# rskew/aiko_services

Measured on AMD Instinct MI355X. Metric: frames/sec (whole node) + p50 latency, ResNet-50 pipeline at 1/2/4/8 MI355X, higher is better.
Workload: dtype bf16; 1 GPU; global_batch=640, per_gpu_batch=640, parallelism=dp1, hipgraph=True, ingest=hbm, setup_frames=12, model=resnet50, pipeline=(SyntheticFrames ResNet50Classifier ClassifierTopK), gpu_lanes=2

## Files before the change

aiko_services_amd/csrc/bindings/conv.cpp:

```cpp
#include "checks.h"

namespace {

void conv_igemm_out(const at::Tensor& x, const c10::optional<at::Tensor>& x2, const at::Tensor& w,
                    const c10::optional<at::Tensor>& bias, const c10::optional<at::Tensor>& res,
                    at::Tensor& y, at::IntArrayRef geom, const c10::optional<at::Tensor>& zero) {
  TORCH_CHECK(geom.size() == 21 || geom.size() == 22, "aiko.conv_igemm_out: geom needs 21 or 22 ints");
  const int64_t variant = geom.size() == 22 ? geom[21] : 0;
  const int64_t H = geom[0], W = geom[1], C = geom[2], Cc = geom[3], R = geom[4], S = geom[5];
  const int64_t stride = geom[6], pad = geom[7], Ho = geom[8], Wo = geom[9], M = geom[10];
  const int64_t act = geom[11], ldy = geom[12], ldr = geom[13], bm = geom[14], bn = geom[15];
  const int64_t K1 = geom[16], H2 = geom[17], W2 = geom[18], C2 = geom[19], stride2 = geom[20];
  check_cuda_all({&x, &w, &y}, {"x", "w", "y"});
  TORCH_CHECK(x.scalar_type() == at::kBFloat16 && w.scalar_type() == at::kBFloat16 &&
                  y.scalar_type() == at::kBFloat16,
              "aiko.conv_igemm_out: x, w, y must be bfloat16");
  TORCH_CHECK(w.dim() == 2 && w.is_contiguous(), "aiko.conv_igemm_out: w must be [Cout, K] contiguous");
  const int64_t Cout = w.size(0), K = w.size(1);
  const bool dual = defined(x2);
  const int64_t Kmain = dual ? K1 : K;
  TORCH_CHECK(Kmain >= R * S * Cc && Kmain % 64 == 0 && Kmain - R * S * Cc < 64, "aiko.conv_igemm_out: K=",
              Kmain, " must be R*S*Cc rounded up to a multiple of 64");
  const void* x2ptr = nullptr;
  if (dual) {
    check_cuda(*x2, "x2");
    TORCH_CHECK(x2->scalar_type() == at::kBFloat16, "aiko.conv_igemm_out: x2 must be bf16");
    TORCH_CHECK((K - K1) % 64 == 0 && K - K1 <= C2 && C2 % 8 == 0 && K1 > 0,
                "aiko.conv_igemm_out: second source needs K-K1 (multiple of 64) <= C2");
    TORCH_CHECK(aligned(*x2, 16), "aiko.conv_igemm_out: x2 alignment");
    TORCH_CHECK(M % (Ho * Wo) == 0 && (Ho - 1) * stride2 < H2 && (Wo - 1) * stride2 < W2 &&
                    avail_elems(*x2) >= (M / (Ho * Wo)) * H2 * W2 * C2,
                "aiko.conv_igemm_out: x2 too small for the output geometry");
    x2ptr = x2->data_ptr();
  }
  TORCH_CHECK(Cc % 8 == 0 && (Cc <= C || C == 4), "aiko.conv_igemm_out: Cc must be a multiple of 8 within the pixel pitch (or span pixels of a 4-channel stem input)");
// ... 435 lines not shown
    dbg_ptr = reinterpret_cast<unsigned*>(dbg->data_ptr());
  }
  TORCH_CHECK(B * H * W * 256 < INT_MAX, "aiko.bneck_fused_out: batch too large for 32-bit pixel indices");
  check_launch(aiko_bneck_fused(x.data_ptr(), w1.data_ptr(), b1.data_ptr<float>(), w2.data_ptr(), b2.data_ptr<float>(),
                                w3.data_ptr(), b3.data_ptr<float>(), y.data_ptr(), (int)B, (int)H, (int)W, (int)cin,
                                (int)grid, dbg_ptr, cur_stream()),
               "bneck_fused");
}

void conv3x3_exp_out(const at::Tensor& t1, const at::Tensor& w2, const at::Tensor& b2, const at::Tensor& w3,
                     const at::Tensor& b3, const at::Tensor& res, at::Tensor& y, int64_t grid) {
  for (const at::Tensor* t : {&t1, &w2, &b2, &w3, &b3, &res, (const at::Tensor*)&y}) {
    check_cuda(*t, "conv3x3_exp operand");
    TORCH_CHECK(t->is_contiguous() && aligned(*t, 16),
                "aiko.conv3x3_exp_out: operands must be contiguous and 16-byte aligned");
  }
  for (const at::Tensor* t : {&t1, &w2, &w3, &res, (const at::Tensor*)&y})
    TORCH_CHECK(t->scalar_type() == at::kBFloat16, "aiko.conv3x3_exp_out: bf16 activations / weights");
  for (const at::Tensor* t : {&b2, &b3})
    TORCH_CHECK(t->scalar_type() == at::kFloat, "aiko.conv3x3_exp_out: fp32 biases");
  TORCH_CHECK(t1.dim() == 4 && t1.size(3) == 256, "aiko.conv3x3_exp_out: t1 must be [B, H, W, 256] NHWC");
  const int64_t B = t1.size(0), H = t1.size(1), W = t1.size(2);
  TORCH_CHECK(y.dim() == 4 && y.size(0) == B && y.size(1) == H && y.size(2) == W, "aiko.conv3x3_exp_out: y must be [B, H, W, N]");
  const int64_t N = y.size(3);
  TORCH_CHECK(N > 0 && N % 256 == 0, "aiko.conv3x3_exp_out: N must be a multiple of 256");
  TORCH_CHECK(res.sizes() == y.sizes(), "aiko.conv3x3_exp_out: res must have y's shape (identity residual)");
  TORCH_CHECK(w2.numel() == 256 * 9 * 256 && w2.size(0) == 256, "aiko.conv3x3_exp_out: w2 [256, 2304] (3x3, tap-major)");
  TORCH_CHECK(w3.numel() == N * 256, "aiko.conv3x3_exp_out: w3 must be the [N / 16, 8, 64, 8] fragment image");
  TORCH_CHECK(b2.numel() == 256 && b3.numel() == N, "aiko.conv3x3_exp_out: biases [256], [N]");
  TORCH_CHECK(y.data_ptr() != res.data_ptr() && y.data_ptr() != t1.data_ptr(), "aiko.conv3x3_exp_out: in place is not supported");
  TORCH_CHECK(grid >= 0, "aiko.conv3x3_exp_out: grid must be >= 0 (0: one workgroup per tile)");
  TORCH_CHECK(B > 0 && H > 0 && W > 0 && B * H * W * N * 2 < 0x7ffffff0LL,
              "aiko.conv3x3_exp_out: tensors too large for 32-bit offsets");
  check_launch(aiko_conv3x3_exp(t1.data_ptr(), w2.data_ptr(), b2.data_ptr<float>(), w3.data_ptr(), b3.data_ptr<float>(),
                                res.data_ptr(), y.data_ptr(), (int)B, (int)H, (int)W, (int)N, (int)grid, cur_stream()),
               "conv3x3_exp");
}

void stem_direct_out(const at::Tensor& frames, const at::Tensor& w, const c10::optional<at::Tensor>& bias,
                     at::Tensor& out, at::IntArrayRef geom, double fill, at::ArrayRef<double> mean,
                     at::ArrayRef<double> std, bool bgr) {
  check_cuda_all({&frames, &w, &out}, {"frames", "w", "out"});
  TORCH_CHECK(frames.scalar_type() == at::kByte && frames.dim() == 4 && frames.size(3) == 3 && frames.is_contiguous(),
              "aiko.stem_direct_out: frames must be uint8 [B, H, W, 3] contiguous");
  TORCH_CHECK(geom.size() == 10, "aiko.stem_direct_out: geom = [Ho, Wo, Hc, Wc, off_t, off_l, k, stride, pad, act]");
  const int64_t Ho = geom[0], Wo = geom[1], Hc = geom[2], Wc = geom[3], off_t = geom[4], off_l = geom[5];
  const int64_t k = geom[6], stride = geom[7], pad = geom[8], act = geom[9];
  TORCH_CHECK(off_t >= 0 && off_l >= 0 && off_t + Ho <= Hc && off_l + Wo <= Wc,
              "aiko.stem_direct_out: image must lie inside the canvas");
  const int64_t B = frames.size(0), Cout = out.size(3);
  const int64_t H1 = (Hc + 2 * pad - k) / stride + 1, W1 = (Wc + 2 * pad - k) / stride + 1;
  TORCH_CHECK(out.size(0) == B && out.size(1) == H1 && out.size(2) == W1, "aiko.stem_direct_out: out must be [B, ",
              H1, ", ", W1, ", Cout]");
  const int64_t ldo = pixel_pitch(out, "stem_direct_out");
  TORCH_CHECK(w.scalar_type() == at::kBFloat16 && w.is_contiguous() && w.dim() == 2 && w.size(0) == Cout &&
                  w.size(1) == 64 && k * k * 4 <= 64 && Cout % 16 == 0,
              "aiko.stem_direct_out: w bf16 [Cout, 64] contiguous (k <= 4, Cout % 16 == 0)");
  const float* bp = nullptr;
  if (defined(bias)) {
    check_cuda(*bias, "bias");
    TORCH_CHECK(bias->scalar_type() == at::kFloat && bias->numel() == Cout && bias->is_contiguous(), "aiko.stem_direct_out: bias fp32 [Cout]");
    bp = bias->data_ptr<float>();
  }
  TORCH_CHECK(mean.size() == 3 && std.size() == 3, "aiko.stem_direct_out: mean/std need 3 values");
  float m[3] = {(float)mean[0], (float)mean[1], (float)mean[2]};
  float s[3] = {(float)std[0], (float)std[1], (float)std[2]};
  check_launch(aiko_stem_direct(frames.data_ptr(), out.data_ptr(), w.data_ptr(), bp, B, frames.size(1),
                                frames.size(2), Ho, Wo, Hc, Wc, off_t, off_l, (float)fill, m, s, bgr ? 1 : 0, H1, W1,
// ... 73 lines not shown
```

aiko_services_amd/csrc/kernels/aiko_api.h:

```cpp
#pragma once

#include <hip/hip_runtime.h>

#include "conv_launch.h"

extern "C" {

int aiko_conv_igemm(const ConvLaunch* l);
int aiko_conv_glds(const ConvLaunch* l, const void* zero);
int aiko_conv_glds_tail(const void* x, const void* w, const float* bias, int H, int W, int C, int Cc, int R, int S,
                        int stride, int pad, int Ho, int Wo, int M, int K, int N, int act, const void* w2, const float* b2,
                        void* y2, int ldy2, int ldw2, int act2, const void* zero, const int* dec, void* boxes,
                        float* scores, int* cls, hipStream_t stream);
int aiko_conv_buf(const ConvLaunch* l, int occ, int mf32);
int aiko_conv_persist(const ConvLaunch* l);
int aiko_conv_wide(const ConvLaunch* l, int occ);

int aiko_conv_pw(const void* x, const void* w, const float* bias, const void* res, void* y, int M, int N,
                 int K, int ldx, int ldy, int ldr, int act, int cus, int mode, hipStream_t stream);
int aiko_conv_pw_dual(const void* x, const void* x2, const void* w, const float* bias, void* y, int M, int N,
                      int ldx, int ldx2, int ldy, int act, int Ho, int Wo, int H2, int W2, int s2, int cus,
                      hipStream_t stream);

int aiko_conv_narrow(const void* x, const void* w, const float* bias, const void* res, void* y, int H, int W, int C,
                     int Cc, int R, int S, int stride, int pad, int Ho, int Wo, int M, int Cout, int K, int act,
                     int ldy, int ldr, int th, int wreg, hipStream_t stream);

int aiko_conv3x3_patch(const void* x, const void* wimg, const float* bias, void* y, int B, int H, int W, int ldy,
                       int act, int grid, hipStream_t stream);
int aiko_conv3x3_patchw(const void* x, const void* wimg, const float* bias, void* y, int B, int H, int W, int ldx,
                        int ldy, int act, int grid, hipStream_t stream);
int aiko_conv3x3_rows(const void* x, const void* wimg, const float* bias, const void* res, void* y, int B, int H,
                      int W, int ldx, int ldy, int ldr, int act, int grid, hipStream_t stream);

int aiko_conv_chain(const void* A, const void* W1, const float* b1, const void* R, void* Y, const void* W2,
                    const float* b2, void* Z, const void* A2, int M, int K1, int N1, int N2, int grid,
                    hipStream_t stream);
int aiko_conv_chain2(const void* A, const void* W1, const float* b1, const void* R, void* Y, const void* W2,
                     const float* b2, void* Z, int M, int K1, int N1, int N2, int grid, hipStream_t stream);

int aiko_bneck_fused(const void* x, const void* w1, const float* b1, const void* w2, const float* b2,
                     const void* w3, const float* b3, void* y, int B, int H, int W, int cin, int grid,
                     unsigned* dbg, hipStream_t stream);
int aiko_conv3x3_exp(const void* t1, const void* w2, const float* b2, const void* w3img, const float* b3,
                     const void* res, void* y, int B, int H, int W, int N, int grid, hipStream_t stream);
int aiko_c2f_fused(const void* x, int ldx, const void* w1, const float* b1, int k1, const void* wa, const float* ba,
                   int ka, const void* wb, const float* bb, int kb, const void* w2, const float* b2, int k2, void* y, int ldy,
                   int B, int H, int W, int CI, int C, int CO, int shortcut, int rb, const void* xu, int ldxu, int cu, hipStream_t stream);
int aiko_c2f_bneck(const void* x, int ldx, const void* wa, const float* ba, int ka, const void* wb, const float* bb,
                   int kb, void* y, int ldy, int B, int H, int W, int C, int shortcut, int rb, hipStream_t stream);

int aiko_stem_pool(const void* x, const void* w, const float* bias, void* y, int B, int Hp, int Wp,
                   int Ho, int Wo, int Hm, int Wm, int ldy, int variant, hipStream_t stream);
int aiko_stem_pool_u8(const void* frames, const void* w, const float* bias, void* y, int B, int Hi, int Wi,
                      int Ho, int Wo, int Hm, int Wm, int ldy, const float* mean255, int variant, hipStream_t stream);

int aiko_resize_u8(const void* in, void* out, int B, int Hin, int Win, int Ho, int Wo, hipStream_t stream);
int aiko_batchnorm(const void* x, void* y, const float* scale, const float* shift, long P, int C, int ldx,
                   int ldy, int act, hipStream_t stream);
int aiko_preprocess(const void* in, void* out, int B, int Hin, int Win, int Ho, int Wo, int Hp,
                    int Wp, int pad_t, int pad_l, int Hc, int Wc, int off_t, int off_l, float fill,
                    const float* mean, const float* std, int bgr, hipStream_t stream);
int aiko_stem_direct(const void* in, void* out, const void* w, const float* bias, int B, int Hin, int Win,
                     int Ho, int Wo, int Hc, int Wc, int off_t, int off_l, float fill, const float* mean,
                     const float* std, int bgr, int H1, int W1, int Cout, int ldo, int k, int stride, int pad,
                     int act, hipStream_t stream);
int aiko_maxpool(const void* x, void* y, int B, int H, int W, int C, int Ho, int Wo, int k,
                 int s, int p, int ldx, int ldy, hipStream_t stream);
int aiko_mean_rows_f32(const void* x, float* y, int B, int T, int C, long ldb, hipStream_t stream);
int aiko_avgpool(const void* x, void* y, int B, int HW, int C, hipStream_t stream);
int aiko_softmax_topk(const void* logits, float* prob, int* index, int B, int N, int k,
                      hipStream_t stream);
int aiko_sppf_pool(void* x, int B, int H, int W, int ld, int c, int k, hipStream_t stream);
int aiko_zero_border_rows(void* x, int B, int rows, int C, hipStream_t stream);

int aiko_upsample2x(const void* x, void* y, int B, int H, int W, int C, int ldx, int ldy,
                    hipStream_t stream);
int aiko_yolo_decode(const void* const* feats, const int* H, const int* W, const int* strides,
// ... 114 lines not shown
```

aiko_services_amd/csrc/kernels/conv_exp.hip:

```cpp
#include <type_traits>

#include "conv_common.h"
#include "conv_wide_stage.h"
#include "aiko_api.h"

namespace aiko {

typedef __attribute__((ext_vector_type(2))) short i16x2;

__device__ __forceinline__ uint32_t relu_bf16x2(uint32_t v) {
  return __builtin_bit_cast(uint32_t, __builtin_elementwise_max(__builtin_bit_cast(i16x2, v), i16x2{0, 0}));
}

struct ConvExpParams {
  ConvParams c;
  const bf16_t* w3;
  const float* b3;
  int N;
};

__global__ __launch_bounds__(512, 1) void conv3x3_exp_kernel(ConvExpParams q) {
  const ConvParams& p = q.c;
  constexpr int BM = 256, BN = 256, BK = 64, WGN = 4, NW = 8, NS = 2;
  constexpr int WM = 128, WN = 64, MI = 8, NI = 4, NP = 2;
  constexpr int RPW = 8, RPI = 64, APT = 4, BPT = 4;
  constexpr int STAGE_ELEMS = (BM + BN) * BK;
  constexpr int T2_BLOCK = BM * 64;
  static_assert(NS * STAGE_ELEMS == 4 * T2_BLOCK, "the t2 slice fills the ring exactly");
  __shared__ __attribute__((aligned(16))) bf16_t ring[NS * STAGE_ELEMS];

  const int wave = __builtin_amdgcn_readfirstlane(threadIdx.x >> 6);
  const int wr = wave / WGN, wc = wave % WGN;
  const int ntiles = (p.M + BM - 1) / BM;
  const int G = gridDim.x;
  const int lid = xcd_remap(blockIdx.x, G);

  const __amdgpu_buffer_rsrc_t rx = wide_rsrc(p.x);
  const __amdgpu_buffer_rsrc_t rw = wide_rsrc(p.w);
  const __amdgpu_buffer_rsrc_t rw3 = wide_rsrc(q.w3);
  const int io_bytes = p.M * q.N * 2;
  const __amdgpu_buffer_rsrc_t rr =
      __builtin_amdgcn_make_buffer_rsrc(const_cast<bf16_t*>(p.res), (short)0, io_bytes, 0x00020000);
  const __amdgpu_buffer_rsrc_t ry = __builtin_amdgcn_make_buffer_rsrc(p.y, (short)0, io_bytes, 0x00020000);

  const int nkb = p.K / BK;
  const int nch = q.N / 128;

  for (int tile = lid; tile < ntiles; tile += G) {
    const int m0 = tile * BM;
    uint32_t lz = 0u;
    asm volatile("" : "+v"(lz));
    const int lane1 = __builtin_amdgcn_mbcnt_hi(~0u, __builtin_amdgcn_mbcnt_lo(~0u, lz));
    const int lrow = wave * RPW + (lane1 >> 3);
    const int lp = (lane1 & 7) ^ (lane1 >> 3);
    const int HoWo = p.Ho * p.Wo;
    uint32_t b_off[BPT];
#pragma unroll
    for (int i = 0; i < BPT; ++i) b_off[i] = (uint32_t)(((lrow + RPI * i) * p.K + lp * 8) * 2);

    const int fr = lane1 & 15, fq = lane1 >> 4;
    const int coff = ((fq & 1) << 4) | ((fq >> 1) << 3);
    const int sw = fr & 7;
// ... 110 lines not shown
      }
      if (kb < nkb) step(kb, S0{});
    }

    uint32_t lz2 = 0u;
    asm volatile("" : "+v"(lz2));
    const int lane2 = __builtin_amdgcn_mbcnt_hi(~0u, __builtin_amdgcn_mbcnt_lo(~0u, lz2));
    const int fr2 = lane2 & 15, fq2 = lane2 >> 4;
    const int coff2 = ((fq2 & 1) << 4) | ((fq2 >> 1) << 3);
    const int sw2 = fr2 & 7;
    const int x_r0 = (wr * WM + fr2) * 64;
    __syncthreads();
#pragma unroll
    for (int i = 0; i < MI; ++i) {
#pragma unroll
      for (int h = 0; h < NP; ++h) {
        f32x4 lo = acc[2 * h][i], hi = acc[2 * h + 1][i];
#pragma unroll
        for (int e = 0; e < 4; ++e) {
          const auto s = __builtin_amdgcn_permlane16_swap(__float_as_uint(lo[e]), __float_as_uint(hi[e]), false, false);
          lo[e] = __uint_as_float(s[0]);
          hi[e] = __uint_as_float(s[1]);
        }
        u32x4 o;
        o[0] = pack2(fmaxf(lo[0] + e_bias[h][0], 0.f), fmaxf(lo[1] + e_bias[h][1], 0.f));
        o[1] = pack2(fmaxf(lo[2] + e_bias[h][2], 0.f), fmaxf(lo[3] + e_bias[h][3], 0.f));
        o[2] = pack2(fmaxf(hi[0] + e_bias[h][4], 0.f), fmaxf(hi[1] + e_bias[h][5], 0.f));
        o[3] = pack2(fmaxf(hi[2] + e_bias[h][6], 0.f), fmaxf(hi[3] + e_bias[h][7], 0.f));
        const int piece = (h * 4 + (coff2 >> 3)) ^ sw2;
        *reinterpret_cast<u32x4*>(ring + wc * T2_BLOCK + (x_r0 + i * 16 * 64) + (piece << 3)) = o;
      }
    }

    const uint32_t row0 = (uint32_t)(((m0 + wr * WM + fr2) * q.N + wc * 32 + coff2) * 2);
    const uint32_t row_step = (uint32_t)(16 * q.N * 2);
    const uint32_t w_off = (uint32_t)(wc * 2 * 8 * 1024 + lane2 * 16);
    bf16x8 wreg[4][2];
    u32x4 e_res[2][MI];
    f32x2 e_b3[4];
    auto load_w = [&](int c, int ks) __attribute__((always_inline)) {
      const uint32_t base = c < nch ? w_off : kWideOOB;
#pragma unroll
      for (int j = 0; j < 2; ++j)
        wreg[ks & 3][j] = __builtin_bit_cast(bf16x8, __builtin_amdgcn_raw_buffer_load_b128(
            rw3, base, (uint32_t)c * 65536u + (uint32_t)((j * 8 + ks) * 1024), 0));
    };
    auto load_res = [&](int c, auto par_tag) __attribute__((always_inline)) {
      constexpr int P = decltype(par_tag)::value;
      const uint32_t cb = (uint32_t)c * 256u;
      const uint32_t base = c < nch ? row0 : kWideOOB;
      uint32_t rs = row_step;
      asm volatile("" : "+s"(rs));
#pragma unroll
      for (int i = 0; i < MI; ++i)
        e_res[P][i] = __builtin_bit_cast(u32x4, __builtin_amdgcn_raw_buffer_load_b128(
            rr, base + rs * i, cb, 0));
    };
    auto load_b3 = [&](int c) __attribute__((always_inline)) {
      const int n = c * 128 + wc * 32 + coff2;
      const f32x4 b0 = *reinterpret_cast<const f32x4*>(q.b3 + n);
      const f32x4 b1 = *reinterpret_cast<const f32x4*>(q.b3 + n + 4);
      e_b3[0] = f32x2{b0[0], b0[1]}; e_b3[1] = f32x2{b0[2], b0[3]};
      e_b3[2] = f32x2{b1[0], b1[1]}; e_b3[3] = f32x2{b1[2], b1[3]};
    };
    using P0 = std::integral_constant<int, 0>;
    using P1 = std::integral_constant<int, 1>;
// ... 47 lines not shown
#pragma unroll
        for (int e = 0; e < 4; ++e) {
          const auto s = __builtin_amdgcn_permlane16_swap(__float_as_uint(lo[e]), __float_as_uint(hi[e]), false, false);
          lo[e] = __uint_as_float(s[0]);
          hi[e] = __uint_as_float(s[1]);
        }
        const f32x2 v[4] = {f32x2{lo[0], lo[1]} + e_b3[0], f32x2{lo[2], lo[3]} + e_b3[1],
                            f32x2{hi[0], hi[1]} + e_b3[2], f32x2{hi[2], hi[3]} + e_b3[3]};
        u32x4 o;
#pragma unroll
        for (int e = 0; e < 4; ++e) {
          const f32x2 r = {__uint_as_float(e_res[P][i][e] << 16), __uint_as_float(e_res[P][i][e] & 0xffff0000u)};
          const f32x2 t = v[e] + r;
          o[e] = relu_bf16x2(pack2(t[0], t[1]));
        }
        __builtin_amdgcn_raw_buffer_store_b128(o, ry, row0 + rs * i, cb, 0);
        asm volatile("s_nop 1");
        __builtin_amdgcn_sched_barrier(0);
      }
      load_res(c + 2, par_tag);
    };
    for (int c = 0; c < nch; c += 2) {
      chunk(c, P0{});
      chunk(c + 1, P1{});
    }
    __syncthreads();
  }
}

}

extern "C" int aiko_conv3x3_exp(const void* t1, const void* w2, const float* b2, const void* w3img,
                                const float* b3, const void* res, void* y, int B, int H, int W, int N,
                                int grid, hipStream_t stream) {
  using namespace aiko;
  const long M = (long)B * H * W;
  if (N <= 0 || N % 256 || M <= 0 || M * N * 2 >= 0x7ffffff0L || H * W <= 0 || grid < 0) return -1;
  ConvExpParams q;
  ConvParams& p = q.c;
  p.x = static_cast<const bf16_t*>(t1);
  p.w = static_cast<const bf16_t*>(w2);
  p.bias = b2;
  p.res = static_cast<const bf16_t*>(res);
  p.y = static_cast<bf16_t*>(y);
  p.H = H; p.W = W; p.C = 256; p.Cc = 256; p.R = 3; p.S = 3;
  p.stride = 1; p.pad = 1; p.Ho = H; p.Wo = W; p.M = (int)M; p.Cout = 256; p.K = 9 * 256;
  p.act = 1; p.ldy = N; p.ldr = N;
  p.x2 = nullptr;
  p.K1 = p.K; p.H2 = 0; p.W2 = 0; p.C2 = 0; p.stride2 = 1;
  conv_params_finalize(p);
  q.w3 = static_cast<const bf16_t*>(w3img);
  q.b3 = b3;
  q.N = N;
  const int ntiles = (int)((M + 255) / 256);
  const int g = grid > 0 && grid < ntiles ? grid : ntiles;
  conv3x3_exp_kernel<<<dim3(g), 512, 0, stream>>>(q);
  return (int)hipGetLastError();
}
```

aiko_services_amd/csrc/kernels/conv_wide.hip:

```cpp
#include <cstdlib>
#include <type_traits>

#include "conv_common.h"
#include "conv_wide_stage.h"
#include "aiko_api.h"

namespace aiko {

template <int BM, int BN, int WGM, int WGN, int NS, bool RES_PF, int OCC, int BK = 64, int NR = 0>
__global__ __launch_bounds__(64 * WGM * WGN, OCC) void conv_wide_kernel(ConvParams p) {
  constexpr int NW = WGM * WGN;
  static_assert(NW == 4 || NW == 8, "4 or 8 waves");
  static_assert(BK == 64 || BK == 32, "64- or 32-deep K blocks");
  constexpr int PPR = BK / 8;
  constexpr int D = NS - 1;
  constexpr int BNR = NR ? NR : BN;
  static_assert(BNR <= BN && BNR % (16 * WGN) == 0, "exact-N tile");
  constexpr int WM = BM / WGM, WN = BNR / WGN;
  constexpr int MI = WM / 16, NI = WN / 16;
  static_assert((NR != 0 || NI % 2 == 0) && MI >= 1, "wave tile: whole 16-pixel blocks, channel blocks in pairs");
  constexpr bool TAIL = NI % 2 != 0;
  constexpr int RPW = 64 / PPR;
  constexpr int RPI = RPW * NW;
  static_assert(BM % RPI == 0 && BN % RPI == 0, "tile rows in whole DMA pieces");
// ... 282 lines not shown
      const f32x4 a = acc[NI - 1][i];
      uint2 r = {0u, 0u};
      if (p.res) {
        if constexpr (RES_PF) r = e_rtail[i];
        else r = *reinterpret_cast<const uint2*>(p.res + (size_t)m * p.ldr + ntail);
      }
      float v[4] = {a[0] + e_btail[0], a[1] + e_btail[1], a[2] + e_btail[2], a[3] + e_btail[3]};
      const float rv[4] = {__uint_as_float(r.x << 16), __uint_as_float(r.x & 0xffff0000u),
                           __uint_as_float(r.y << 16), __uint_as_float(r.y & 0xffff0000u)};
      if (p.res && !post) {
#pragma unroll
        for (int e = 0; e < 4; ++e) v[e] += rv[e];
      }
      if (act == 1) {
#pragma unroll
        for (int e = 0; e < 4; ++e) v[e] = fmaxf(v[e], 0.f);
      } else if (act == 2) {
#pragma unroll
        for (int e = 0; e < 4; ++e) v[e] = silu(v[e]);
      } else if (act == 3) {
#pragma unroll
        for (int e = 0; e < 4; ++e) v[e] = gelu_erf(v[e]);
      }
      if (p.res && post) {
#pragma unroll
        for (int e = 0; e < 4; ++e) v[e] += rv[e];
      }
      *reinterpret_cast<uint2*>(p.y + (size_t)m * p.ldy + ntail) = uint2{pack2(v[0], v[1]), pack2(v[2], v[3])};
    }
  }
}


template <int BM, int BN, int WGM, int WGN, int NS, bool RES = false>
__global__ __launch_bounds__(64 * WGM * WGN, 1) void conv_wide_pers_kernel(ConvParams p) {
  constexpr int BK = 64, PPR = 8;
  constexpr int NW = WGM * WGN;
  static_assert(NW == 8, "8 waves");
  static_assert(NS == 2 || NS == 3, "2- or 3-slot ring");
  constexpr int D = NS - 1;
  constexpr int WM = BM / WGM, WN = BN / WGN;
  constexpr int MI = WM / 16, NI = WN / 16, NP = NI / 2;
  static_assert(NI % 2 == 0, "channel blocks in pairs");
  constexpr int RPW = 64 / PPR, RPI = RPW * NW;
  static_assert(BM % RPI == 0 && BN % RPI == 0, "tile rows in whole DMA pieces");
  constexpr int APT = BM / RPI, BPT = BN / RPI, PER = APT + BPT;
  constexpr int NST = MI * NP;
  constexpr int STAGE_ELEMS = (BM + BN) * BK;
  constexpr int BIAS_FLOATS = 2048;
  static_assert(NS * STAGE_ELEMS * 2 + BIAS_FLOATS * 4 <= 160 * 1024, "LDS budget");
  __shared__ __attribute__((aligned(16))) bf16_t ring[NS * STAGE_ELEMS + BIAS_FLOATS * 2];
  float* const sbias = reinterpret_cast<float*>(ring + NS * STAGE_ELEMS);

  const int tid = threadIdx.x, lane = tid & 63;
  const int wave = __builtin_amdgcn_readfirstlane(tid >> 6);
  const int wr = wave / WGN, wc = wave % WGN;
  const int ntn = (p.Cout + BN - 1) / BN;
  const int ntiles = ((p.M + BM - 1) / BM) * ntn;
  const int G = gridDim.x;
  const int lid = xcd_remap(blockIdx.x, G);
  if (lid >= ntiles) return;
  const int nkb = p.K / BK;
  const int nblocks = ((ntiles - lid + G - 1) / G) * nkb;

  for (int c = tid; c < BIAS_FLOATS; c += 64 * NW) sbias[c] = (p.bias && c < p.Cout) ? p.bias[c] : 0.f;
  __syncthreads();

// ... 216 lines not shown
    }
    if constexpr (RES) {
      if (ckb == nkb - 1 - D) load_res(ct);
    }
    issue_next(std::integral_constant<int, PREV>{});
    compute(slot_tag);
    epi_prev2 = epi_prev;
    epi_prev = false;
    if (++ckb == nkb) {
      epilogue(ct);
      ct += G;
      ckb = 0;
      epi_prev = true;
    }
  };
  int g = 0;
  if constexpr (NS == 2) {
    for (; g + 2 <= nblocks; g += 2) {
      step(g, S0{});
      step(g + 1, S1{});
    }
    if (g < nblocks) step(g, S0{});
  } else {
    for (; g + 3 <= nblocks; g += 3) {
      step(g, S0{});
      step(g + 1, S1{});
      step(g + 2, S2{});
    }
    if (g < nblocks) step(g, S0{});
    if (g + 1 < nblocks) step(g + 1, S1{});
  }
  asm volatile("s_waitcnt vmcnt(0)" ::: "memory");
}
}

extern "C" int aiko_conv_wide(const ConvLaunch* l, int occ) {
  using namespace aiko;
  const int M = l->M, Cout = l->Cout, K = l->K, bm = l->bm, bn = l->bn;
  const void* res = l->res;
  hipStream_t stream = l->stream;
  if (l->Cc % 64 || l->R * l->S > 32 || l->R > 16 || l->S > 16 || (l->x2 && (K - l->K1) % 64) || Cout % 8) return -1;
  const ConvParams p = conv_params(*l);
  dim3 grid(((M + bm - 1) / bm) * ((Cout + bn - 1) / bn));
  if (occ == 18) {
    if (Cout % 16) return -1;
    if (bm == 256 && bn == 80)
      conv_wide_kernel<256, 128, 8, 1, 2, true, 1, 64, 80><<<grid, 512, 0, stream>>>(p);
    else if (bm == 128 && bn == 80)
      conv_wide_kernel<128, 128, 8, 1, 2, true, 2, 64, 80><<<grid, 512, 0, stream>>>(p);
    else if (bm == 256 && bn == 144)
      conv_wide_kernel<256, 192, 8, 1, 2, true, 1, 64, 144><<<grid, 512, 0, stream>>>(p);
    else if (bm == 128 && bn == 144)
      conv_wide_kernel<128, 192, 8, 1, 2, true, 1, 64, 144><<<grid, 512, 0, stream>>>(p);
    else
      return -1;
  } else if (occ == 20) {
    if (Cout > 2048 || (res != nullptr && K < 192)) return -1;
    int dev = 0, cus = 0;
    (void)hipGetDevice(&dev);
    if (hipDeviceGetAttribute(&cus, hipDeviceAttributeMultiprocessorCount, dev) != hipSuccess || cus <= 0) cus = 256;
    const char* cap = getenv("AIKO_CONV_PERS_GRID");
    if (cap && atoi(cap) > 0) cus = atoi(cap);
    const int ntiles = (int)grid.x;
    dim3 pg(ntiles < cus ? ntiles : cus);
    const bool r = res != nullptr;
    if (bm == 256 && bn == 256 && !r)
      conv_wide_pers_kernel<256, 256, 2, 4, 2><<<pg, 512, 0, stream>>>(p);
    else if (bm == 256 && bn == 128 && !r)
      conv_wide_pers_kernel<256, 128, 4, 2, 3><<<pg, 512, 0, stream>>>(p);
    else if (bm == 128 && bn == 256 && !r)
      conv_wide_pers_kernel<128, 256, 2, 4, 3><<<pg, 512, 0, stream>>>(p);
    else if (bm == 256 && bn == 128)
      conv_wide_pers_kernel<256, 128, 4, 2, 3, true><<<pg, 512, 0, stream>>>(p);
    else if (bm == 128 && bn == 256)
      conv_wide_pers_kernel<128, 256, 2, 4, 3, true><<<pg, 512, 0, stream>>>(p);
    else
      return -1;
  } else if (occ == 19) {
    if (bm == 128 && bn == 128)
      conv_wide_kernel<128, 128, 2, 2, 2, true, 2><<<grid, 256, 0, stream>>>(p);
    else if (bm == 128 && bn == 256)
      conv_wide_kernel<128, 256, 2, 2, 3, true, 1><<<grid, 256, 0, stream>>>(p);
    else
      return -1;
  } else if (occ <= 1) {
    if (bm == 256 && bn == 256)
      conv_wide_kernel<256, 256, 2, 4, 2, false, 1><<<grid, 512, 0, stream>>>(p);
    else if (bm == 256 && bn == 128)
      conv_wide_kernel<256, 128, 4, 2, 3, true, 1><<<grid, 512, 0, stream>>>(p);
    else if (bm == 128 && bn == 256)
      conv_wide_kernel<128, 256, 2, 4, 3, true, 1><<<grid, 512, 0, stream>>>(p);
    else if (bm == 256 && bn == 64)
      conv_wide_kernel<256, 64, 4, 2, 3, true, 1><<<grid, 512, 0, stream>>>(p);
    else if (bm == 128 && bn == 128)
      conv_wide_kernel<128, 128, 2, 4, 3, true, 1><<<grid, 512, 0, stream>>>(p);
    else
      return -1;
  } else if (occ == 11) {
    if (bm == 256 && bn == 256)
      conv_wide_kernel<256, 256, 2, 4, 4, false, 1, 32><<<grid, 512, 0, stream>>>(p);
    else if (bm == 256 && bn == 128)
      conv_wide_kernel<256, 128, 4, 2, 4, true, 1, 32><<<grid, 512, 0, stream>>>(p);
    else if (bm == 128 && bn == 256)
      conv_wide_kernel<128, 256, 2, 4, 4, true, 1, 32><<<grid, 512, 0, stream>>>(p);
    else
      return -1;
  } else {
    if (bm == 128 && bn == 128)
// ... 15 lines not shown
```

Baseline: 101,200 frames/s.

## Add register-resident t2 schedule for fused 3x3+expand conv second GEMM

Adds a templated P2REG variant of the fused conv3x3+1x1-expand kernel that loads each wave's t2 activation slice into registers once. The expand weights are then streamed into the LDS ring in double-buffered halves via DMA, and the bias is staged in shared memory. This reorganizes the second GEMM so every wave covers 32 pixel rows across all output channels, aiming to cut repeated LDS activation reads and overlap weight loads with MFMA work. It is enabled by default through an env-var switch for N<=4096, at the cost of more register pressure and extra LDS for the bias.

```diff
diff --git a/aiko_services_amd/csrc/bindings/conv.cpp b/aiko_services_amd/csrc/bindings/conv.cpp
--- a/aiko_services_amd/csrc/bindings/conv.cpp
+++ b/aiko_services_amd/csrc/bindings/conv.cpp
@@ -1,6 +1,8 @@
 #include "checks.h"
 
 namespace {
+
+constexpr int kExpP2Default = 1;
 
 void conv_igemm_out(const at::Tensor& x, const c10::optional<at::Tensor>& x2, const at::Tensor& w,
                     const c10::optional<at::Tensor>& bias, const c10::optional<at::Tensor>& res,
@@ -502,8 +504,14 @@
   TORCH_CHECK(grid >= 0, "aiko.conv3x3_exp_out: grid must be >= 0 (0: one workgroup per tile)");
   TORCH_CHECK(B > 0 && H > 0 && W > 0 && B * H * W * N * 2 < 0x7ffffff0LL,
               "aiko.conv3x3_exp_out: tensors too large for 32-bit offsets");
+  const char* p2 = getenv("AIKO_EXP_P2");
+  int sched = p2 && *p2 ? atoi(p2) : kExpP2Default;
+  TORCH_CHECK(sched == 0 || sched == 1, "aiko.conv3x3_exp_out: AIKO_EXP_P2 must be 0 or 1");
+  if (!(p2 && *p2) && N > 4096) sched = 0;
+  TORCH_CHECK(sched == 0 || N <= 4096, "aiko.conv3x3_exp_out: AIKO_EXP_P2=1 needs N <= 4096");
   check_launch(aiko_conv3x3_exp(t1.data_ptr(), w2.data_ptr(), b2.data_ptr<float>(), w3.data_ptr(), b3.data_ptr<float>(),
-                                res.data_ptr(), y.data_ptr(), (int)B, (int)H, (int)W, (int)N, (int)grid, cur_stream()),
+                                res.data_ptr(), y.data_ptr(), (int)B, (int)H, (int)W, (int)N, (int)grid, sched,
+                                cur_stream()),
                "conv3x3_exp");
 }
 
diff --git a/aiko_services_amd/csrc/kernels/aiko_api.h b/aiko_services_amd/csrc/kernels/aiko_api.h
--- a/aiko_services_amd/csrc/kernels/aiko_api.h
+++ b/aiko_services_amd/csrc/kernels/aiko_api.h
@@ -43,7 +43,7 @@
                      const void* w3, const float* b3, void* y, int B, int H, int W, int cin, int grid,
                      unsigned* dbg, hipStream_t stream);
 int aiko_conv3x3_exp(const void* t1, const void* w2, const float* b2, const void* w3img, const float* b3,
-                     const void* res, void* y, int B, int H, int W, int N, int grid, hipStream_t stream);
+                     const void* res, void* y, int B, int H, int W, int N, int grid, int sched, hipStream_t stream);
 int aiko_c2f_fused(const void* x, int ldx, const void* w1, const float* b1, int k1, const void* wa, const float* ba,
                    int ka, const void* wb, const float* bb, int kb, const void* w2, const float* b2, int k2, void* y, int ldy,
                    int B, int H, int W, int CI, int C, int CO, int shortcut, int rb, const void* xu, int ldxu, int cu, hipStream_t stream);
diff --git a/aiko_services_amd/csrc/kernels/conv_exp.hip b/aiko_services_amd/csrc/kernels/conv_exp.hip
--- a/aiko_services_amd/csrc/kernels/conv_exp.hip
+++ b/aiko_services_amd/csrc/kernels/conv_exp.hip
@@ -19,6 +19,9 @@
   int N;
 };
 
+constexpr int kExpP2MaxN = 4096;
+
+template <bool P2REG>
 __global__ __launch_bounds__(512, 1) void conv3x3_exp_kernel(ConvExpParams q) {
   const ConvParams& p = q.c;
   constexpr int BM = 256, BN = 256, BK = 64, WGN = 4, NW = 8, NS = 2;
@@ -27,7 +30,12 @@
   constexpr int STAGE_ELEMS = (BM + BN) * BK;
   constexpr int T2_BLOCK = BM * 64;
   static_assert(NS * STAGE_ELEMS == 4 * T2_BLOCK, "the t2 slice fills the ring exactly");
-  __shared__ __attribute__((aligned(16))) bf16_t ring[NS * STAGE_ELEMS];
+  constexpr int W3_HALF = NS * STAGE_ELEMS / 2;
+  __shared__ __attribute__((aligned(16))) bf16_t ring[NS * STAGE_ELEMS + (P2REG ? kExpP2MaxN * 2 : 0)];
+  float* b3s = reinterpret_cast<float*>(ring + NS * STAGE_ELEMS);
+  if constexpr (P2REG) {
+    for (int n = threadIdx.x; n < q.N; n += 512) b3s[n] = q.b3[n];
+  }
 
   const int wave = __builtin_amdgcn_readfirstlane(threadIdx.x >> 6);
   const int wr = wave / WGN, wc = wave % WGN;
@@ -204,6 +212,132 @@
       }
     }
 
+    if constexpr (P2REG) {
+      const int px0 = wave * 32 + fr2;
+      const uint32_t row0 = ((uint32_t)(m0 + px0) * (uint32_t)q.N + (uint32_t)coff2) * 2u;
+      const uint32_t row_step = (uint32_t)(16 * q.N * 2);
+      asm volatile("s_waitcnt lgkmcnt(0)\n\ts_barrier" ::: "memory");
+      bf16x8 xt[2][8];
+#pragma unroll
+      for (int pb = 0; pb < 2; ++pb)
+#pragma unroll
+        for (int ks = 0; ks < 8; ++ks)
+          xt[pb][ks] = *reinterpret_cast<const bf16x8*>(
+              ring + (ks >> 1) * T2_BLOCK + (px0 + pb * 16) * 64 + (((((ks & 1) << 2) + fq2) ^ sw2) << 3));
+      asm volatile("s_waitcnt lgkmcnt(0)\n\ts_barrier" ::: "memory");
+
+      const uint32_t w_voff = (uint32_t)(lane2 * 16);
+      auto issue_w = [&](int c, auto half_tag) __attribute__((always_inline)) {
+        constexpr int HALF = decltype(half_tag)::value;
+        if (c < nch) {
+          const uint32_t sb = (uint32_t)c * 65536u + (uint32_t)(wave * 8192);
+#pragma unroll
+          for (int i = 0; i < 8; ++i)
+            wide_dma16(rw3, w_voff, sb + (uint32_t)(i * 1024), ring + HALF * W3_HALF + wave * 4096 + i * 512);
+        }
+        asm volatile("" ::: "memory");
+        __builtin_amdgcn_sched_barrier(0);
+      };
+      u32x4 e_res[2][8];
+      auto load_res = [&](int c, auto par_tag) __attribute__((always_inline)) {
+        constexpr int P = decltype(par_tag)::value;
+        const uint32_t cb = (uint32_t)c * 256u;
+        const uint32_t base = c < nch ? row0 : kWideOOB;
+        uint32_t rs = row_step;
+        asm volatile("" : "+s"(rs));
+#pragma unroll
+        for (int pb = 0; pb < 2; ++pb)
+#pragma unroll
+          for (int j = 0; j < 4; ++j)
+            e_res[P][pb * 4 + j] = __builtin_bit_cast(u32x4, __builtin_amdgcn_raw_buffer_load_b128(
+                rr, base + rs * pb + (uint32_t)(j * 64), cb, 0));
+      };
+      const bf16_t* wa = ring + lane2 * 8;
+      const float* ba = b3s + coff2;
+      f32x4 acc2[8][2];
+      auto kloop = [&](auto half_tag) __attribute__((always_inline)) {
+        constexpr int HALF = decltype(half_tag)::value;
+        const bf16_t* wh = wa + HALF * W3_HALF;
+        auto read_a = [&](int t) __attribute__((always_inline)) {
+          return *reinterpret_cast<const bf16x8*>(wh + (t & 7) * 4096 + (t >> 3) * 512);
+        };
+#pragma unroll
+        for (int nb = 0; nb < 8; ++nb)
+#pragma unroll
+          for (int pb = 0; pb < 2; ++pb) acc2[nb][pb] = f32x4{0.f, 0.f, 0.f, 0.f};
+        constexpr int AW = 6;
+        bf16x8 af[AW];
+#pragma unroll
+        for (int t = 0; t < AW; ++t) af[t] = read_a(t);
+#pragma unroll
+        for (int t = 0; t < 64; ++t) {
+          const int ks = t >> 3, nb = t & 7;
+#pragma unroll
+          for (int pb = 0; pb < 2; ++pb)
+            acc2[nb][pb] = __builtin_amdgcn_mfma_f32_16x16x32_bf16(af[t % AW], xt[pb][ks], acc2[nb][pb], 0, 0, 0);
+          if (t + AW < 64) af[t % AW] = read_a(t + AW);
+          __builtin_amdgcn_sched_barrier(0);
+        }
+      };
+      auto epilogue = [&](int c, auto par_tag) __attribute__((always_inline)) {
+        constexpr int P = decltype(par_tag)::value;
+        const uint32_t cb = (uint32_t)c * 256u;
+        uint32_t rs = row_step;
+        asm volatile("" : "+s"(rs));
+#pragma unroll
+        for (int j = 0; j < 4; ++j) {
+          const f32x4 b0 = *reinterpret_cast<const f32x4*>(ba + c * 128 + j * 32);
+          const f32x4 b1 = *reinterpret_cast<const f32x4*>(ba + c * 128 + j * 32 + 4);
+          const f32x2 e_b3[4] = {f32x2{b0[0], b0[1]}, f32x2{b0[2], b0[3]}, f32x2{b1[0], b1[1]}, f32x2{b1[2], b1[3]}};
+#pragma unroll
+          for (int pb = 0; pb < 2; ++pb) {
+            f32x4 lo = acc2[2 * j][pb], hi = acc2[2 * j + 1][pb];
+#pragma unroll
+            for (int e = 0; e < 4; ++e) {
+              const auto s = __builtin_amdgcn_permlane16_swap(__float_as_uint(lo[e]), __float_as_uint(hi[e]), false, false);
+              lo[e] = __uint_as_float(s[0]);
+              hi[e] = __uint_as_float(s[1]);
+            }
+            const f32x2 v[4] = {f32x2{lo[0], lo[1]} + e_b3[0], f32x2{lo[2], lo[3]} + e_b3[1],
+                                f32x2{hi[0], hi[1]} + e_b3[2], f32x2{hi[2], hi[3]} + e_b3[3]};
+            u32x4 o;
+#pragma unroll
+            for (int e = 0; e < 4; ++e) {
+              const uint32_t rv = e_res[P][pb * 4 + j][e];
+              const f32x2 r = {__uint_as_float(rv << 16), __uint_as_float(rv & 0xffff0000u)};
+              const f32x2 t = v[e] + r;
+              o[e] = relu_bf16x2(pack2(t[0], t[1]));
+            }
+            __builtin_amdgcn_raw_buffer_store_b128(o, ry, row0 + rs * pb + (uint32_t)(j * 64), cb, 0);
+            asm volatile("s_nop 1");
+            __builtin_amdgcn_sched_barrier(0);
+          }
+        }
+        load_res(c + 2, par_tag);
+      };
+      auto publish = [&](int c, auto half_tag) __attribute__((always_inline)) {
+        asm volatile("s_waitcnt vmcnt(16)\n\ts_waitcnt lgkmcnt(0)\n\ts_barrier" ::: "memory");
+        issue_w(c + 2, half_tag);
+      };
+      auto chunk = [&](int c, auto par_tag) __attribute__((always_inline)) {
+        kloop(par_tag);
+        publish(c, par_tag);
+        epilogue(c, par_tag);
+      };
+      using P0 = std::integral_constant<int, 0>;
+      using P1 = std::integral_constant<int, 1>;
+      issue_w(0, P0{});
+      issue_w(1, P1{});
+      load_res(0, P0{});
+      load_res(1, P1{});
+      asm volatile("s_waitcnt vmcnt(24)\n\ts_barrier" ::: "memory");
+      for (int c = 0; c < nch; c += 2) {
+        chunk(c, P0{});
+        chunk(c + 1, P1{});
+      }
+      continue;
+    }
+
     const uint32_t row0 = (uint32_t)(((m0 + wr * WM + fr2) * q.N + wc * 32 + coff2) * 2);
     const uint32_t row_step = (uint32_t)(16 * q.N * 2);
     const uint32_t w_off = (uint32_t)(wc * 2 * 8 * 1024 + lane2 * 16);
@@ -317,10 +451,11 @@
 
 extern "C" int aiko_conv3x3_exp(const void* t1, const void* w2, const float* b2, const void* w3img,
                                 const float* b3, const void* res, void* y, int B, int H, int W, int N,
-                                int grid, hipStream_t stream) {
+                                int grid, int sched, hipStream_t stream) {
   using namespace aiko;
   const long M = (long)B * H * W;
   if (N <= 0 || N % 256 || M <= 0 || M * N * 2 >= 0x7ffffff0L || H * W <= 0 || grid < 0) return -1;
+  if ((sched != 0 && sched != 1) || (sched == 1 && N > kExpP2MaxN)) return -1;
   ConvExpParams q;
   ConvParams& p = q.c;
   p.x = static_cast<const bf16_t*>(t1);
@@ -339,6 +474,7 @@
   q.N = N;
   const int ntiles = (int)((M + 255) / 256);
   const int g = grid > 0 && grid < ntiles ? grid : ntiles;
-  conv3x3_exp_kernel<<<dim3(g), 512, 0, stream>>>(q);
+  if (sched == 1) conv3x3_exp_kernel<true><<<dim3(g), 512, 0, stream>>>(q);
+  else conv3x3_exp_kernel<false><<<dim3(g), 512, 0, stream>>>(q);
   return (int)hipGetLastError();
 }
```

After: 102,000 frames/s, median of 6. No clear change (+0.8%).

## Add lean persistent wide-conv kernel specialized for activation and pointwise convs

Applied to the files above, without the earlier changes.

Adds a compile-time specialized persistent conv kernel variant where the activation (none or ReLU) and a pointwise (1x1, stride 1, no pad) fast path are template parameters. The pointwise path skips per-tap im2col address and mask setup, and ReLU is applied as a packed bf16 integer max after packing. It is enabled by default through an environment switch, and the 256x128 non-residual tile is excluded from the pointwise path. The cost is more template instantiations and code size, plus separate code paths that must stay numerically consistent with the generic kernel.

```diff
diff --git a/aiko_services_amd/csrc/kernels/conv_wide.hip b/aiko_services_amd/csrc/kernels/conv_wide.hip
--- a/aiko_services_amd/csrc/kernels/conv_wide.hip
+++ b/aiko_services_amd/csrc/kernels/conv_wide.hip
@@ -338,7 +338,8 @@
 }
 
 
-template <int BM, int BN, int WGM, int WGN, int NS, bool RES = false>
+template <int BM, int BN, int WGM, int WGN, int NS, bool RES = false, int ACT = -1, bool PW = false,
+          std::enable_if_t<(ACT < 0), int> = 0>
 __global__ __launch_bounds__(64 * WGM * WGN, 1) void conv_wide_pers_kernel(ConvParams p) {
   constexpr int BK = 64, PPR = 8;
   constexpr int NW = WGM * WGN;
@@ -621,6 +622,327 @@
   }
   asm volatile("s_waitcnt vmcnt(0)" ::: "memory");
 }
+
+__device__ __forceinline__ uint32_t wide_relu2(uint32_t v) {
+  typedef short s16x2 __attribute__((ext_vector_type(2)));
+  const s16x2 r = __builtin_elementwise_max(__builtin_bit_cast(s16x2, v), s16x2{0, 0});
+  return __builtin_bit_cast(uint32_t, r);
+}
+
+template <int BM, int BN, int WGM, int WGN, int NS, bool RES, int ACT, bool PW>
+__device__ __forceinline__ void wide_pers_lean(const ConvParams& p) {
+  static_assert(ACT == 0 || ACT == 1, "none or ReLU");
+  constexpr int BK = 64, PPR = 8;
+  constexpr int NW = WGM * WGN;
+  static_assert(NW == 8, "8 waves");
+  static_assert(NS == 2 || NS == 3, "2- or 3-slot ring");
+  constexpr int D = NS - 1;
+  constexpr int WM = BM / WGM, WN = BN / WGN;
+  constexpr int MI = WM / 16, NI = WN / 16, NP = NI / 2;
+  static_assert(NI % 2 == 0, "channel blocks in pairs");
+  constexpr int RPW = 64 / PPR, RPI = RPW * NW;
+  static_assert(BM % RPI == 0 && BN % RPI == 0, "tile rows in whole DMA pieces");
+  constexpr int APT = BM / RPI, BPT = BN / RPI, PER = APT + BPT;
+  constexpr int NST = MI * NP;
+  constexpr int STAGE_ELEMS = (BM + BN) * BK;
+  constexpr int BIAS_FLOATS = 2048;
+  static_assert(NS * STAGE_ELEMS * 2 + BIAS_FLOATS * 4 <= 160 * 1024 && BIAS_FLOATS % BN == 0, "LDS budget");
+  __shared__ __attribute__((aligned(16))) bf16_t ring[NS * STAGE_ELEMS + BIAS_FLOATS * 2];
+  float* const sbias = reinterpret_cast<float*>(ring + NS * STAGE_ELEMS);
+
+  const int tid = threadIdx.x, lane = tid & 63;
+  const int wave = __builtin_amdgcn_readfirstlane(tid >> 6);
+  const int wr = wave / WGN, wc = wave % WGN;
+  const int ntn = (p.Cout + BN - 1) / BN, ntm = (p.M + BM - 1) / BM;
+  const int G = gridDim.x;
+  const int lid = xcd_remap(blockIdx.x, G);
+  if (lid >= ntm * ntn) return;
+  const int nkb = p.K / BK;
+  const int Gq = G / ntn, Gr = G - Gq * ntn;
+  const int tm0 = lid / ntn, tn0 = lid - tm0 * ntn;
+  auto advance = [&](int& tm, int& tn) __attribute__((always_inline)) {
+    tm += Gq;
+    tn += Gr;
+    if (tn >= ntn) {
+      tn -= ntn;
+      ++tm;
+    }
+  };
+
+  for (int c = tid; c < BIAS_FLOATS; c += 64 * NW) sbias[c] = (p.bias && c < p.Cout) ? p.bias[c] : 0.f;
+  __syncthreads();
+
+  const int lrow = wave * RPW + lane / PPR;
+  const int lp = (lane & 7) ^ (lane >> 3);
+  const __amdgpu_buffer_rsrc_t rx = wide_rsrc(p.x);
+  const __amdgpu_buffer_rsrc_t rw = wide_rsrc(p.w);
+  const __amdgpu_buffer_rsrc_t rx2 = wide_rsrc(p.x2 ? p.x2 : p.x);
+  const __amdgpu_buffer_rsrc_t ry = wide_rsrc(p.y);
+  const __amdgpu_buffer_rsrc_t rr = wide_rsrc(p.res ? p.res : p.y);
+
+  int itm = tm0, itn = tn0, ikb = 0;
+  uint32_t a_off[APT], b_off[BPT];
+  const uint32_t a_lin = (uint32_t)((lrow * p.C + lp * 8) * 2);
+  const uint32_t b_lin = (uint32_t)((lrow * p.K + lp * 8) * 2);
+  int a_base[APT];
+  uint32_t a_mask[APT], a2_off[APT];
+  int cur_tap = -1, iss_tap = 0, iss_c = 0, iss_r = 0, iss_s = 0;
+  const int K1 = p.x2 ? p.K1 : p.K;
+  const int HoWo = p.Ho * p.Wo;
+  auto setup_issue = [&]() __attribute__((always_inline)) {
+    const int m0 = itm * BM, n0 = itn * BN;
+    if constexpr (PW) {
+      const int rows = p.M - m0 - lrow;
+#pragma unroll
+      for (int i = 0; i < APT; ++i)
+        a_off[i] = RPI * i < rows ? a_lin + (uint32_t)(m0 + RPI * i) * (uint32_t)(p.C * 2) : kWideOOB;
+    } else {
+#pragma unroll
+      for (int i = 0; i < APT; ++i) {
+        const int m = m0 + lrow + RPI * i;
+        a_mask[i] = 0u;
+        a_base[i] = 0;
+        a2_off[i] = kWideOOB;
+        a_off[i] = kWideOOB;
+        if (m < p.M) {
+          const int img = fdiv(m, p.mHoWo, p.lHoWo);
+          const int rem = m - img * HoWo;
+          const int oh = fdiv(rem, p.mWo, p.lWo);
+          const int ow = rem - oh * p.Wo;
+          const int ih0 = oh * p.stride - p.pad, iw0 = ow * p.stride - p.pad;
+          a_base[i] = (((img * p.H + ih0) * p.W + iw0) * p.C + lp * 8) * 2;
+          const int r_lo = max(0, -ih0), r_hi = min(p.R, p.H - ih0);
+          const int s_lo = max(0, -iw0), s_hi = min(p.S, p.W - iw0);
+          const uint32_t mr = r_hi > r_lo ? ((1u << r_hi) - 1u) & ~((1u << r_lo) - 1u) : 0u;
+          const uint32_t ms = s_hi > s_lo ? ((1u << s_hi) - 1u) & ~((1u << s_lo) - 1u) : 0u;
+          a_mask[i] = mr | (ms << 16);
+          a2_off[i] = (uint32_t)((((img * p.H2 + oh * p.stride2) * p.W2 + ow * p.stride2) * p.C2 + lp * 8) * 2);
+        }
+      }
+      cur_tap = -1;
+      iss_tap = iss_c = iss_r = iss_s = 0;
+    }
+    const int cols = p.Cout - n0 - lrow;
+#pragma unroll
+    for (int i = 0; i < BPT; ++i)
+      b_off[i] = RPI * i < cols ? b_lin + (uint32_t)(n0 + RPI * i) * (uint32_t)(p.K * 2) : kWideOOB;
+  };
+  auto issue_next = [&](auto slot_tag) __attribute__((always_inline)) {
+    constexpr int SLOT = decltype(slot_tag)::value;
+    if (itm >= ntm) return false;
+    bf16_t* Xs = ring + SLOT * STAGE_ELEMS;
+    bf16_t* Ws = Xs + BM * BK;
+    const int k0 = ikb * BK;
+    const uint32_t sb = (uint32_t)(k0 * 2);
+#pragma unroll
+    for (int i = 0; i < BPT; ++i) wide_dma16(rw, b_off[i], sb, Ws + (i * RPI + wave * RPW) * BK);
+    if constexpr (PW) {
+#pragma unroll
+      for (int i = 0; i < APT; ++i) wide_dma16(rx, a_off[i], sb, Xs + (i * RPI + wave * RPW) * BK);
+    } else if (k0 >= K1) {
+      const uint32_t soff = (uint32_t)((k0 - K1) * 2);
+#pragma unroll
+      for (int i = 0; i < APT; ++i) wide_dma16(rx2, a2_off[i], soff, Xs + (i * RPI + wave * RPW) * BK);
+    } else {
+      if (iss_tap != cur_tap) {
+        cur_tap = iss_tap;
+        const int tap_off = ((iss_r * p.W + iss_s) * p.C) * 2;
+        const uint32_t bit = (1u << iss_r) | (1u << (iss_s + 16));
+#pragma unroll
+        for (int i = 0; i < APT; ++i)
+          a_off[i] = (a_mask[i] & bit) == bit ? (uint32_t)(a_base[i] + tap_off) : kWideOOB;
+      }
+      const uint32_t soff = (uint32_t)(iss_c * 2);
+#pragma unroll
+      for (int i = 0; i < APT; ++i) wide_dma16(rx, a_off[i], soff, Xs + (i * RPI + wave * RPW) * BK);
+      iss_c += BK;
+      if (iss_c >= p.Cc) {
+        iss_c = 0;
+        ++iss_tap;
+        if (++iss_s == p.S) {
+          iss_s = 0;
+          ++iss_r;
+        }
+      }
+    }
+    if (++ikb == nkb) {
+      ikb = 0;
+      advance(itm, itn);
+      if (itm < ntm) setup_issue();
+    }
+    return true;
+  };
+
+  const int fr = lane & 15, fq = lane >> 4;
+  const int coff = ((fq & 1) << 4) | ((fq >> 1) << 3);
+  const int sw = fr & 7;
+  int w_rd[NI], x_rd[MI];
+#pragma unroll
+  for (int j = 0; j < NI; ++j) w_rd[j] = BM * BK + (wc * WN + j * 16 + fr) * BK;
+#pragma unroll
+  for (int i = 0; i < MI; ++i) x_rd[i] = (wr * WM + i * 16 + fr) * BK;
+  f32x4 acc[NI][MI];
+#pragma unroll
+  for (int j = 0; j < NI; ++j)
+#pragma unroll
+    for (int i = 0; i < MI; ++i) acc[j][i] = f32x4{0.f, 0.f, 0.f, 0.f};
+  auto compute = [&](auto slot_tag) __attribute__((always_inline)) {
+    constexpr int SLOT = decltype(slot_tag)::value;
+    const bf16_t* St = ring + SLOT * STAGE_ELEMS;
+#pragma unroll
+    for (int kk = 0; kk < BK / 32; ++kk) {
+      const int pc = ((fq + 4 * kk) ^ sw) << 3;
+      bf16x8 wf[NI], xf[MI];
+#pragma unroll
+      for (int j = 0; j < NI; ++j) wf[j] = *reinterpret_cast<const bf16x8*>(St + w_rd[j] + pc);
+#pragma unroll
+      for (int i = 0; i < MI; ++i) xf[i] = *reinterpret_cast<const bf16x8*>(St + x_rd[i] + pc);
+#pragma unroll
+      for (int i = 0; i < MI; ++i)
+#pragma unroll
+        for (int j = 0; j < NI; ++j)
+          acc[j][i] = __builtin_amdgcn_mfma_f32_16x16x32_bf16(wf[j], xf[i], acc[j][i], 0, 0, 0);
+    }
+  };
+  int ctm = tm0, ctn = tn0, ckb = 0;
+  const int e_row = wr * WM + fr, e_col = wc * WN + coff;
+  const uint32_t y_lin = (uint32_t)((e_row * p.ldy + e_col) * 2);
+  const uint32_t r_lin = (uint32_t)((e_row * p.ldr + e_col) * 2);
+  u32x4 e_res[RES ? MI : 1][RES ? NP : 1];
+  auto load_res = [&]() __attribute__((always_inline)) {
+    const int m0 = ctm * BM, n0 = ctn * BN;
+    const int rows = p.M - m0 - e_row;
+    const uint32_t off = r_lin + (uint32_t)(m0 * p.ldr + n0) * 2u;
+    uint32_t cflag[NP];
+#pragma unroll
+    for (int q = 0; q < NP; ++q) cflag[q] = n0 + e_col + 32 * q < p.Cout ? 0u : kWideOOB;
+#pragma unroll
+    for (int i = 0; i < MI; ++i) {
+      const uint32_t roff = 16 * i < rows ? off + (uint32_t)(16 * i) * (uint32_t)(p.ldr * 2) : kWideOOB;
+#pragma unroll
+      for (int q = 0; q < NP; ++q)
+        e_res[i][q] = __builtin_bit_cast(u32x4, __builtin_amdgcn_raw_buffer_load_b128(rr, roff | cflag[q], 64 * q, 0));
+    }
+  };
+  auto epilogue = [&]() __attribute__((always_inline)) {
+    const int m0 = ctm * BM, n0 = ctn * BN;
+    const int rows = p.M - m0 - e_row;
+    const uint32_t off = y_lin + (uint32_t)(m0 * p.ldy + n0) * 2u;
+    uint32_t cflag[NP];
+    f32x4 b0[NP], b1[NP];
+#pragma unroll
+    for (int q = 0; q < NP; ++q) {
+      cflag[q] = n0 + e_col + 32 * q < p.Cout ? 0u : kWideOOB;
+      const float* b = sbias + n0 + wc * WN + 32 * q + (RES ? coff : 4 * fq);
+      b0[q] = *reinterpret_cast<const f32x4*>(b);
+      b1[q] = *reinterpret_cast<const f32x4*>(b + (RES ? 4 : 16));
+    }
+#pragma unroll
+    for (int i = 0; i < MI; ++i) {
+      const uint32_t roff = 16 * i < rows ? off + (uint32_t)(16 * i) * (uint32_t)(p.ldy * 2) : kWideOOB;
+#pragma unroll
+      for (int q = 0; q < NP; ++q) {
+        f32x4 lo = acc[2 * q][i], hi = acc[2 * q + 1][i];
+        u32x4 o;
+        if constexpr (RES) {
+#pragma unroll
+          for (int e = 0; e < 4; ++e) {
+            const auto s2 = __builtin_amdgcn_permlane16_swap(__float_as_uint(lo[e]), __float_as_uint(hi[e]), false, false);
+            lo[e] = __uint_as_float(s2[0]);
+            hi[e] = __uint_as_float(s2[1]);
+          }
+          float v[8] = {lo[0] + b0[q][0], lo[1] + b0[q][1], lo[2] + b0[q][2], lo[3] + b0[q][3],
+                        hi[0] + b1[q][0], hi[1] + b1[q][1], hi[2] + b1[q][2], hi[3] + b1[q][3]};
+#pragma unroll
+          for (int e = 0; e < 4; ++e) {
+            v[2 * e] += __uint_as_float(e_res[i][q][e] << 16);
+            v[2 * e + 1] += __uint_as_float(e_res[i][q][e] & 0xffff0000u);
+            o[e] = pack2(v[2 * e], v[2 * e + 1]);
+          }
+        } else {
+          const uint32_t l0 = pack2(lo[0] + b0[q][0], lo[1] + b0[q][1]), l1 = pack2(lo[2] + b0[q][2], lo[3] + b0[q][3]);
+          const uint32_t h0 = pack2(hi[0] + b1[q][0], hi[1] + b1[q][1]), h1 = pack2(hi[2] + b1[q][2], hi[3] + b1[q][3]);
+          const auto s0 = __builtin_amdgcn_permlane16_swap(l0, h0, false, false);
+          const auto s1 = __builtin_amdgcn_permlane16_swap(l1, h1, false, false);
+          o = u32x4{s0[0], s1[0], s0[1], s1[1]};
+        }
+        if constexpr (ACT == 1) {
+#pragma unroll
+          for (int e = 0; e < 4; ++e) o[e] = wide_relu2(o[e]);
+        }
+        __builtin_amdgcn_raw_buffer_store_b128(o, ry, roff | cflag[q], 64 * q, 0);
+      }
+    }
+#pragma unroll
+    for (int j = 0; j < NI; ++j)
+#pragma unroll
+      for (int i = 0; i < MI; ++i) acc[j][i] = f32x4{0.f, 0.f, 0.f, 0.f};
+  };
+
+  setup_issue();
+  using S0 = std::integral_constant<int, 0>;
+  using S1 = std::integral_constant<int, 1>;
+  using S2 = std::integral_constant<int, 2>;
+  int ahead = 0;
+  ahead += issue_next(S0{});
+  if constexpr (NS == 3) ahead += issue_next(S1{});
+  bool epi_prev = false;
+  bool epi_prev2 = false;
+  auto step = [&](auto slot_tag) __attribute__((always_inline)) {
+    constexpr int SLOT = decltype(slot_tag)::value;
+    constexpr int PREV = SLOT == 0 ? NS - 1 : SLOT - 1;
+    if constexpr (D == 1) {
+      if (epi_prev) wide_vm_barrier<NST>();
+      else wide_vm_barrier<0>();
+    } else {
+      const bool more = ahead > 1;
+      const bool epi = epi_prev || epi_prev2;
+      if (more && epi) wide_vm_barrier<PER + NST>();
+      else if (more) wide_vm_barrier<PER>();
+      else if (epi) wide_vm_barrier<NST>();
+      else wide_vm_barrier<0>();
+    }
+    --ahead;
+    if constexpr (RES) {
+      if (ckb == nkb - 1 - D) load_res();
+    }
+    ahead += issue_next(std::integral_constant<int, PREV>{});
+    compute(slot_tag);
+    epi_prev2 = epi_prev;
+    epi_prev = false;
+    if (++ckb == nkb) {
+      epilogue();
+      advance(ctm, ctn);
+      ckb = 0;
+      epi_prev = true;
+      return ctm >= ntm;
+    }
+    return false;
+  };
+  for (;;) {
+    if (step(S0{})) break;
+    if (step(S1{})) break;
+    if constexpr (NS == 3) {
+      if (step(S2{})) break;
+    }
+  }
+  asm volatile("s_waitcnt vmcnt(0)" ::: "memory");
+}
+
+template <int BM, int BN, int WGM, int WGN, int NS, bool RES, int ACT, bool PW, std::enable_if_t<(ACT >= 0), int> = 0>
+__global__ __launch_bounds__(64 * WGM * WGN, 1) void conv_wide_pers_kernel(ConvParams p) {
+  wide_pers_lean<BM, BN, WGM, WGN, NS, RES, ACT, PW>(p);
+}
+}
+
+template <int BM, int BN, int WGM, int WGN, int NS, bool RES>
+static void launch_wide_pers(const aiko::ConvParams& p, dim3 grid, hipStream_t stream, int act, bool pw) {
+  using namespace aiko;
+  if (act == 0 && pw) conv_wide_pers_kernel<BM, BN, WGM, WGN, NS, RES, 0, true><<<grid, 512, 0, stream>>>(p);
+  else if (act == 0) conv_wide_pers_kernel<BM, BN, WGM, WGN, NS, RES, 0, false><<<grid, 512, 0, stream>>>(p);
+  else if (act == 1 && pw) conv_wide_pers_kernel<BM, BN, WGM, WGN, NS, RES, 1, true><<<grid, 512, 0, stream>>>(p);
+  else if (act == 1) conv_wide_pers_kernel<BM, BN, WGM, WGN, NS, RES, 1, false><<<grid, 512, 0, stream>>>(p);
+  else conv_wide_pers_kernel<BM, BN, WGM, WGN, NS, RES><<<grid, 512, 0, stream>>>(p);
 }
 
 extern "C" int aiko_conv_wide(const ConvLaunch* l, int occ) {
@@ -653,16 +975,22 @@
     const int ntiles = (int)grid.x;
     dim3 pg(ntiles < cus ? ntiles : cus);
     const bool r = res != nullptr;
+    const char* lean = getenv("AIKO_WIDE_PERS_LEAN");
+    const int lean_mode = lean ? atoi(lean) : 1;
+    const int act = lean_mode == 0 || l->act > 1 ? -1 : l->act;
+    const bool pw = lean_mode != 2 && (lean_mode == 3 || !(bm == 256 && bn == 128 && !r)) && l->R == 1 &&
+                    l->S == 1 && l->stride == 1 && l->pad == 0 && !l->x2 && l->Ho == l->H && l->Wo == l->W &&
+                    l->Cc == K;
     if (bm == 256 && bn == 256 && !r)
-      conv_wide_pers_kernel<256, 256, 2, 4, 2><<<pg, 512, 0, stream>>>(p);
+      launch_wide_pers<256, 256, 2, 4, 2, false>(p, pg, stream, act, pw);
     else if (bm == 256 && bn == 128 && !r)
-      conv_wide_pers_kernel<256, 128, 4, 2, 3><<<pg, 512, 0, stream>>>(p);
+      launch_wide_pers<256, 128, 4, 2, 3, false>(p, pg, stream, act, pw);
     else if (bm == 128 && bn == 256 && !r)
-      conv_wide_pers_kernel<128, 256, 2, 4, 3><<<pg, 512, 0, stream>>>(p);
+      launch_wide_pers<128, 256, 2, 4, 3, false>(p, pg, stream, act, pw);
     else if (bm == 256 && bn == 128)
-      conv_wide_pers_kernel<256, 128, 4, 2, 3, true><<<pg, 512, 0, stream>>>(p);
+      launch_wide_pers<256, 128, 4, 2, 3, true>(p, pg, stream, act, pw);
     else if (bm == 128 && bn == 256)
-      conv_wide_pers_kernel<128, 256, 2, 4, 3, true><<<pg, 512, 0, stream>>>(p);
+      launch_wide_pers<128, 256, 2, 4, 3, true>(p, pg, stream, act, pw);
     else
       return -1;
   } else if (occ == 19) {
```

Result: slower. 101,700 frames/s before, 99840 frames/s after (-1.8%).
